# eanswer/TactileSimulation

Hardware: AMD Instinct MI355X
Metric: env-steps/sec (fwd+bwd) TactilePush batch=4096 (higher is better)
Workload: dtype f32

## Files before the change

include/tsim.h:

```cpp
#ifndef TSIM_H
#define TSIM_H
#include <stdint.h>
#ifdef __cplusplus
extern "C" {
#endif

typedef struct tsim_batch tsim_batch;
enum { TSIM_F32 = 0, TSIM_F64 = 1 };

int tsim_batch_create(const int32_t* I, const double* F, int B, int tape_capacity, int dtype, int device,
                      tsim_batch** out);
void tsim_batch_destroy(tsim_batch* b);

int tsim_ndof_r(const tsim_batch* b);
int tsim_ndof_u(const tsim_batch* b);
int tsim_ndof_var(const tsim_batch* b);
int tsim_ndof_tactile(const tsim_batch* b);
int tsim_batch_size(const tsim_batch* b);
int tsim_dtype(const tsim_batch* b);
double tsim_timestep(const tsim_batch* b);
int tsim_tape_len(const tsim_batch* b);

int tsim_update_model(tsim_batch* b, const int32_t* I, const double* F, void* stream);

// ... 53 lines not shown

int tsim_cache_save(tsim_batch* b, void* stream);
int tsim_cache_pop(tsim_batch* b, void* stream);
int tsim_cache_clear(tsim_batch* b);
int tsim_cache_reserve(tsim_batch* b, int depth);
int tsim_cache_depth(const tsim_batch* b);

int tsim_debug_eval(tsim_batch* b, const void* q1, const void* q0, const void* qd0, const void* u,
                    void* g_out, void* H_out, long long* cycles, void* stream);

int tsim_debug_signature(tsim_batch* b, int t_first, int n, uint32_t* out, void* stream);

int tsim_debug_stamps(tsim_batch* b, long long* cycles);

int tsim_launch_info(const tsim_batch* b, int32_t* out);
enum { TSIM_KT_FORWARD = 0, TSIM_KT_TAXELS = 1, TSIM_KT_BACKWARD = 2, TSIM_KT_COUNT = 3 };
int tsim_kernel_timing(tsim_batch* b, int enable);
int tsim_kernel_times(tsim_batch* b, double* ms_sum, int32_t* launches);
int tsim_set_lanes_per_env(tsim_batch* b, int lanes);
int tsim_static_model(const tsim_batch* b);
int tsim_set_static(tsim_batch* b, int allow);
const char* tsim_kernel_variant(const tsim_batch* b);
enum { TSIM_OPT_PAIR_CULL = 1, TSIM_OPT_VALUE_TRIALS = 2, TSIM_OPT_TRIAL_HELPERS = 3, TSIM_OPT_VALUE_FIRST = 4, TSIM_OPT_CROSS_KINKS = 5, TSIM_OPT_EVAL_BUDGET = 6,
       TSIM_OPT_ALL_DEFAULT = 7, TSIM_OPT_FRAME_RECORDS = 8, TSIM_OPT_FORWARD_SPLIT = 9, TSIM_OPT_PREDICTOR_HELPERS = 10 };
int tsim_set_option(tsim_batch* b, int option, int value);
int tsim_get_option(const tsim_batch* b, int option);

int tsim_last_evals(tsim_batch* b, int32_t* host_out);
int tsim_last_helper_trials(tsim_batch* b, int32_t* host_out);

#define TSIM_KINK_FACTOR 1000.0
#define TSIM_KINK_LS 4
#define TSIM_KINK_MAX 6
int tsim_set_solver_options(tsim_batch* b, int cross_kinks, int eval_budget);
int tsim_last_gnorm(tsim_batch* b, float* host_out);

const char* tsim_last_error(void);

#ifdef __cplusplus
}
#endif
#endif
```

tactilesimulation_amd/csrc/tsim_batch.h:

```cpp
#pragma once
#include <hip/hip_runtime.h>
#include <cstdint>
#include <string>
#include <vector>
#include "../../include/tsim.h"
#include "tsim_launch.h"

static thread_local std::string g_err;
static int fail(const std::string& m) { g_err = m; return 1; }
#define HIPCHK(x) do { hipError_t e_ = (x); if (e_ != hipSuccess) return fail(std::string(#x) + ": " + hipGetErrorString(e_)); } while (0)

struct DeviceGuard {
  int prev = -1; bool ok = true;
  explicit DeviceGuard(int dev) {
    if (hipGetDevice(&prev) != hipSuccess) prev = -1;
    if (prev != dev) ok = hipSetDevice(dev) == hipSuccess; else prev = -1;
  }
  ~DeviceGuard() { if (prev >= 0) (void)hipSetDevice(prev); }
};
#define TS_DEVICE(b) DeviceGuard guard_((b)->device); if (!guard_.ok) return fail("hipSetDevice(" + std::to_string((b)->device) + ") failed")

static bool capturing(hipStream_t st) {
  hipStreamCaptureStatus cs = hipStreamCaptureStatusNone;
  return hipStreamIsCapturing(st, &cs) != hipSuccess || cs != hipStreamCaptureStatusNone;
// ... 47 lines not shown
  int value_trials = 2;
  int pred_helpers = 1;
  int trial_helpers = 1;
  int value_first = 1;
  bool ab_no_episode_lpt = false, ab_inkernel_readout = false, ab_no_free_run = false, ab_lockstep = false, ab_taxels_per_record = false, ab_no_envtab_cpt = false, ab_no_default_opts = false, ab_inkernel_frame_out = false; int ab_bwd_lpe = 0, ab_lpt_deal = 2;
  int pair_cull = 1;
  int static_id = 0, static_exact = 0, env_struct_ok = 0, no_static = 0;
  DevBuf dKmask, dFlag;
  DevBuf fposeR, fposeD; int fpose_frames = 0;
  int pose_valid = 0;
  int pose_off = 0;
  int tt_off = 0;
  int tax_slots = 0;
  size_t esz;
  std::vector<CacheEntry> cache;
  std::vector<void*> pool;
  std::vector<void*> retired;
  long long* bwd_stamps = nullptr;
  void* dLdp = nullptr; DevBuf zbuf, pgpart; int pg_chunks = 0;
  int pg_groups = TS_PG_CONTACT; DevBuf pgbpart;
  DevBuf tan_src; size_t tan_src_reals = 0; int tan_src_captured = 0;
  DevBuf pg_slots;
  int adj_kernel = -1, adj_passes = 0;
  int kt_on = 0;
  std::vector<KtPair> kt;
  std::vector<hipEvent_t> kt_free;
};
template <class F> static auto by_real(const tsim_batch* b, F&& f) { return by_dtype(b->dtype, f); }
static void split_release(tsim_batch* b) {
  if (b->split_st) (void)hipStreamDestroy(b->split_st);
  if (b->split_fork) (void)hipEventDestroy(b->split_fork);
  if (b->split_join) (void)hipEventDestroy(b->split_join);
  b->split_st = nullptr; b->split_fork = b->split_join = nullptr;
}

struct KtScope {
  tsim_batch* b; hipStream_t st; KtPair p; bool on = false;
  KtScope(tsim_batch* b_, int kind, hipStream_t st_) : b(b_), st(st_) {
    if (!b->kt_on || b->kt.size() >= (size_t)1 << 16) return;
    if (capturing(st)) return;
    hipEvent_t e[2];
    for (int i = 0; i < 2; ++i) {
      if (!b->kt_free.empty()) { e[i] = b->kt_free.back(); b->kt_free.pop_back(); }
      else if (hipEventCreate(&e[i]) != hipSuccess) { (void)hipGetLastError(); if (i) b->kt_free.push_back(e[0]); return; }
    }
    p.a = e[0]; p.b = e[1]; p.kind = kind;
// ... 27 lines not shown
```

tactilesimulation_amd/csrc/tsim_env_push.h:

```cpp
#pragma once

template <class R>
__global__ void __launch_bounds__(256) k_push_action(int B, const R* __restrict__ u, const R* __restrict__ ext, R* __restrict__ a) {
  const int i = blockIdx.x * 256 + threadIdx.x;
  if (i >= B * 6) return;
  const int e = i / 6, c = i - e * 6;
  a[i] = c < 3 ? (R)tanh((double)u[e * 3 + c]) : (c < 5 ? ext[e * 2 + c - 3] : (R)0);
}

template <class R>
__global__ void __launch_bounds__(256) k_push_action_bwd(int B, const R* __restrict__ u, const R* __restrict__ da, R* __restrict__ du) {
  const int i = blockIdx.x * 256 + threadIdx.x;
  if (i >= B * 3) return;
  const int e = i / 3, c = i - e * 3;
  const double t = tanh((double)u[i]);
  du[i] = (R)((double)da[e * 6 + c] * (1.0 - t * t));
}

template <class R>
__global__ void __launch_bounds__(256) k_push_observe(int B, int ntac, const R* __restrict__ q, const R* __restrict__ var,
                                                      const R* __restrict__ tac, const R* __restrict__ goal, const R* __restrict__ u,
                                                      R* __restrict__ obs, R* __restrict__ rew) {
  const int W = 3 + ntac;
  const long long i = (long long)blockIdx.x * 256 + threadIdx.x;
// ... 145 lines not shown
  if (pol->obs_mode == TSIM_PUSH_OBS_TACTILE && (!tac0 || !tac_out)) return fail("push_closed_rollout: tac0 and tac_out are required with the tactile observation (they feed it)");
  if (b->record && b->t_cur + (long long)num_frames * num_steps > b->cap) return fail("push_closed_rollout: tape capacity exceeded (" + std::to_string(b->cap) + " sub-steps)");
  TS_DEVICE(b);
  if (int rc = by_real(b, [&](auto r) { return push_closed_rollout_t<decltype(r)>(b, pol, goal, dist, tac0, num_frames, num_steps, q_out, qd_out, var_out, tac_out, u_out, gl_out, h1_out, h2_out, status, (hipStream_t)stream); })) return rc;
  if (b->record) b->t_cur += num_frames * num_steps;
  b->has_prev = 1;
  return 0;
}

template <class R>
static int push_closed_backward_t(tsim_batch* b, const tsim_push_policy* pol, const void* goal, int nframes, int nsub, const void* df_dq, const void* df_dvar,
                                  const void* du_direct, const void* u_out, const void* h1_out, const void* h2_out, void* g1_out, void* g2_out, void* g3_out,
                                  void* dobs_tac, void* df_du, hipStream_t st) {
  BwdArgs<R> a = bwd_args<R>(b);
  a.n = nframes * nsub; a.seed_stride = nsub; a.frames = 1;
  a.df_dq = (const R*)df_dq; a.df_dvar = (const R*)df_dvar; a.df_du = (R*)df_du;
  a.pol = make_push_policy<R>(pol);
  a.pol.goal = (const R*)goal; a.pol.du_direct = (const R*)du_direct;
  a.pol.u_out = (R*)u_out; a.pol.h1_out = (R*)h1_out; a.pol.h2_out = (R*)h2_out;
  a.pol.g1_out = (R*)g1_out; a.pol.g2_out = (R*)g2_out; a.pol.g3_out = (R*)g3_out; a.pol.dobs_tac = (R*)dobs_tac;
  if (!ts_launch<true, R>(ts_plan(b, b->dLdp ? TS_K_CLOSED_BACKWARD_Z : TS_K_BACKWARD, true, 0), st, a, (R*)b->zbuf)) return fail("no closed-loop k_backward instantiation for the launch plan");
  HIPCHK(hipGetLastError());
  b->adj_kernel = b->dLdp ? TSIM_ADJ_CLOSED_BACKWARD_Z : TSIM_ADJ_BACKWARD;
  if (!b->dLdp) { b->adj_passes = 0; return 0; }
  const R* seeds = nullptr;
  if (a.pol.mode == TSIM_PUSH_OBS_TACTILE && (b->pg_groups & TS_PG_CONTACT)) {
    if (nframes > b->cap || !b->pg_slots) return fail("push_closed_backward: the seed table is missing or too small");
    ts_closed_slots_launch(b->pg_slots, nframes, st);
    HIPCHK(hipGetLastError());
    seeds = (const R*)dobs_tac + (size_t)b->B * PP_NTAC;
  }
  return launch_param_passes<R>(b, a.n, nsub, 1, seeds ? (const int32_t*)b->pg_slots : nullptr, seeds, st);
}

extern "C" int tsim_push_closed_backward(tsim_batch* b, const tsim_push_policy* pol, const void* goal, int num_frames, int num_steps,
                                         const void* df_dq, const void* df_dvar, const void* du_direct, const void* u_out, const void* h1_out, const void* h2_out,
                                         void* g1_out, void* g2_out, void* g3_out, void* dobs_tac, void* df_du, void* stream) {
  if (int rc = push_closed_check(b, pol, num_frames, num_steps, "push_closed_backward")) return rc;
  if (!pol->W1p || !pol->W2 || pol->w1_stride < push_obs_len(pol->obs_mode) || pol->w1_stride % 4 || pol->w1_stride > 64 * (int)PP_OCH) return fail("push_closed_backward: W1p [64][w1_stride >= observation length, multiple of 4] and W2 are required");
  if (!b->record) return fail("push_closed_backward: reset(backward_flag=True) was not called");
  long long n;
  if (int rc = taped_window(b, "push_closed_backward", num_frames, num_steps, &n)) return rc;
  if (!goal || !du_direct || !u_out || !h1_out || !h2_out || !g1_out || !g2_out || !g3_out) return fail("push_closed_backward: null pointer");
  if (pol->obs_mode == TSIM_PUSH_OBS_TACTILE && !dobs_tac) return fail("push_closed_backward: dobs_tac is required with the tactile observation");
  TS_DEVICE(b);
  if (int rc = by_real(b, [&](auto r) { return push_closed_backward_t<decltype(r)>(b, pol, goal, num_frames, num_steps, df_dq, df_dvar, du_direct, u_out, h1_out, h2_out, g1_out, g2_out, g3_out, dobs_tac, df_du, (hipStream_t)stream); })) return rc;
// ... 48 lines not shown
```

tactilesimulation_amd/csrc/tsim_hip.hip:

```cpp
#include <hip/hip_runtime.h>
#include <cstdio>
#include <cstdlib>
#include <cstring>
#include <cmath>
#include <algorithm>
#include <string>
#include <vector>
#include "../../include/tsim.h"
#include "tsim_eval.h"
#include "tsim_policy_push.h"
#include "tsim_static_pusher.h"


#include "tsim_kernels.h"
#include "tsim_param_grad.h"
#include "tsim_launch.h"
#include "tsim_batch.h"

__global__ void __launch_bounds__(1024) k_order_by_evals(const int* evals, int* order, int B, int ns, int lo, int span, int deal) {
  __shared__ int hist[64], base[64];
  const int t = threadIdx.x;
  if (t < 64) hist[t] = 0;
  __syncthreads();
  auto bin = [lo, span](int ev) { return min(max((ev - lo) * 64 / span, 0), 63); };
  for (int e = t; e < B; e += 1024) atomicAdd(&hist[bin(evals[e])], 1);
  __syncthreads();
  if (t == 0) { int acc = 0; for (int k = 63; k >= 0; --k) { base[k] = acc; acc += hist[k]; } }
  __syncthreads();
  const int nwaves = (B + ns - 1) / ns;
  for (int e = t; e < B; e += 1024) {
    const int r = atomicAdd(&base[bin(evals[e])], 1);
    int w = r % nwaves;
    const int sl = r / nwaves;
    if ((deal == 1 && (sl & 1)) || (deal == 2 && sl > 0)) w = nwaves - 1 - w;
    order[w * ns + sl] = e;
  }
}

template <class R> struct ReadArgs { const int* I; const R* F; const R* Fenv; int fstride; int B, t0; const R* tape; R* var_out; R* poseR; double* poseD; int nspt; int stage_cpt; int tk; };
// ... 748 lines not shown
template <class R>
static int launch_param_passes(tsim_batch* b, int n, int seed_stride, int frames, const int32_t* tac_slot, const void* df_dtac, hipStream_t st) {
  b->adj_passes = 0;
  if (!b->dLdp) return 0;
  if (b->pg_groups & TS_PG_CONTACT) {
    if (launch_param_grad<R>(b, n, seed_stride, frames, tac_slot, df_dtac, st)) return 1;
    b->adj_passes |= 1;
  }
  if (b->pg_groups & ~TS_PG_CONTACT) {
    if (launch_param_grad_body<R>(b, n, st)) return 1;
    b->adj_passes |= 2;
  }
  return 0;
}

template <class R>
static int launch_backward(tsim_batch* b, int n, int seed_stride, int frames, const int32_t* tac_slot, const void* df_dq, const void* df_dvar, const void* df_dtac, void* df_du, hipStream_t st) {
  BwdArgs<R> a = bwd_args<R>(b);
  a.n = n; a.seed_stride = seed_stride; a.frames = frames; a.tac_slot = tac_slot;
  a.df_dq = (const R*)df_dq; a.df_dvar = (const R*)df_dvar; a.df_dtac = (const R*)df_dtac; a.df_du = (R*)df_du; a.cyc = b->bwd_stamps;
  {
    KtScope kt_(b, TSIM_KT_BACKWARD, st);
    const TsPlan plan = ts_plan(b, b->dLdp ? TS_K_BACKWARD_Z : TS_K_BACKWARD, false, b->ab_bwd_lpe);
    if (!ts_launch<false, R>(plan, st, a, (R*)b->zbuf)) return fail("no k_backward instantiation for the launch plan");
  }
  HIPCHK(hipGetLastError());
  b->adj_kernel = b->dLdp ? TSIM_ADJ_BACKWARD_Z : TSIM_ADJ_BACKWARD;
  return launch_param_passes<R>(b, n, seed_stride, frames, tac_slot, df_dtac, st);
}

static SlotPlan tangent_plan(const tsim_batch* b, int ndir, bool with_dtab, int kernel = TS_K_TANGENT) {
  const int nhist = b->I[TSIM_IH_INTEGRATOR] == 2 ? 4 : 2, P = with_dtab ? ts_pg_count(b->I[TSIM_IH_NPAIR], b->I[TSIM_IH_NSENSOR], b->nr) : 0;
  return slot_block_plan(b, ts_plan(b, kernel, false, 0), 0, ts_tan_slot_reals(b->nr, b->nu, P, nhist, ndir));
}
template <class R>
static void tangent_args(const tsim_batch* b, TanArgs<R>& a, int T, int S, int ndir, const int32_t* tac_slot, const void* du, const void* dq0, const void* dqd0, const void* dtab,
                         void* dq_out, void* dqd_out, void* dvar_out, void* dtac_out) {
  a.I = b->dI; a.F = (const R*)b->dF; a.Fenv = (const R*)b->dFenv; a.fstride = b->nfrec;
  a.B = b->B; a.n = T * S; a.t_end = b->t_cur; a.nsub = S; a.nframes = T; a.ndir = ndir; a.tk = b->tape_k;
  a.stage_cpt = b->stage_cpt; a.cull = b->pair_cull; a.tac_slot = tac_slot; a.tape = (const R*)b->tape;
  a.du = (const R*)du; a.dq0 = (const R*)dq0; a.dqd0 = (const R*)dqd0; a.dtab = (const R*)dtab;
  a.dq_out = (R*)dq_out; a.dqd_out = (R*)dqd_out; a.dvar_out = (R*)dvar_out; a.dtac_out = (R*)dtac_out;
}
template <class R>
static int launch_tangent_body_src(tsim_batch* b, TanArgs<R>& a, hipStream_t st, const char* who) {
  if (!a.dtab || !(b->pg_groups & ~TS_PG_CONTACT)) return 0;
  const int ndir = a.ndir;
// ... 176 lines not shown
  {
    int cus = 0;
    if (hipDeviceGetAttribute(&cus, hipDeviceAttributeMultiprocessorCount, device) != hipSuccess || cus <= 0) cus = 256;
    b->n_simd = 4 * cus;
  }
  b->stage_cpt = 0;
  detect_static_model(b);
  b->tape_k = kernel_mode(b, b->lpe_forced) != TS_KM_GENERIC ? 1 : 0;
  b->rec = ts_rec(nr, nu, (int)b->esz, b->tape_k);
  if (lds_bytes_for(b, 1) > 64 * 1024) { delete b; return fail("model needs more than 64 KiB of LDS per environment"); }
  decide_stage_cpt(b);
  b->nspt = b->I[TSIM_IH_NSPRIM];
  size_t tape_bytes = (size_t)(tape_capacity + 1) * B * b->rec * b->esz;
  if (hipMalloc(&b->dI, (b->I.size() + b->nsched) * sizeof(int32_t)) != hipSuccess || hipMalloc(&b->dF, b->F.size() * b->esz) != hipSuccess ||
      hipMalloc(&b->tape, tape_bytes) != hipSuccess || hipMalloc(&b->lamq, (size_t)2 * B * nr * b->esz) != hipSuccess ||
      hipMalloc(&b->lamv, (size_t)2 * B * nr * b->esz) != hipSuccess || hipMalloc(&b->evals, (size_t)B * sizeof(int)) != hipSuccess || hipMalloc((void**)&b->helped, (size_t)B * sizeof(int)) != hipSuccess || hipMemset(b->helped, 0, (size_t)B * sizeof(int)) != hipSuccess || hipMalloc((void**)&b->gnorm, (size_t)B * sizeof(float)) != hipSuccess || hipMalloc(&b->order, (size_t)B * sizeof(int)) != hipSuccess || hipMalloc((void**)&b->order_ep, (size_t)B * sizeof(int)) != hipSuccess || hipMalloc(&b->prev, (size_t)B * 2 * nr * sizeof(double)) != hipSuccess ||
      (b->nspt > 0 && (hipMalloc(&b->poseR, (size_t)B * b->nspt * TP_R_SIZE * b->esz) != hipSuccess || hipMalloc((void**)&b->poseD, (size_t)B * b->nspt * TP_D_SIZE * sizeof(double)) != hipSuccess))) {
    tsim_batch_destroy(b);
    return fail("hipMalloc failed (tape bytes = " + std::to_string(tape_bytes) + ")");
  }
  if (hipMemset(b->tape, 0, tape_bytes) != hipSuccess || hipMemset(b->lamq, 0, (size_t)2 * B * nr * b->esz) != hipSuccess ||
      hipMemset(b->lamv, 0, (size_t)2 * B * nr * b->esz) != hipSuccess) { tsim_batch_destroy(b); return fail("hipMemset failed"); }
  if (upload_model(b, nullptr)) { tsim_batch_destroy(b); return 1; }
  if (B >= 64 && !getenv("TSIM_NO_FORWARD_SPLIT")) {
    if (hipStreamCreateWithFlags(&b->split_st, hipStreamNonBlocking) != hipSuccess || hipEventCreateWithFlags(&b->split_fork, hipEventDisableTiming) != hipSuccess ||
        hipEventCreateWithFlags(&b->split_join, hipEventDisableTiming) != hipSuccess) {
      (void)hipGetLastError();
      split_release(b);
    }
  }
  *out = b;
  return 0;
}

void tsim_batch_destroy(tsim_batch* b) {
  if (!b) return;
  DeviceGuard guard_(b->device);
  for (auto& e : b->cache) (void)hipFree(e.buf);
  for (void* p : b->pool) (void)hipFree(p);
  for (void* p : b->retired) (void)hipFree(p);
  for (auto& k : b->kt) { (void)hipEventDestroy(k.a); (void)hipEventDestroy(k.b); }
  for (hipEvent_t e : b->kt_free) (void)hipEventDestroy(e);
  split_release(b);
  (void)hipFree(b->tape);
  delete b;
}
// ... 47 lines not shown
  if (lanes != 0 && lanes != 16 && lanes != 32 && lanes != 64) return fail("set_lanes_per_env: 0 (automatic), 16, 32 or 64");
  b->lpe_forced = lanes;
  shape_changed(b);
  return 0;
}
int tsim_static_model(const tsim_batch* b) { return kernel_mode(b, b->lpe_forced) != TS_KM_GENERIC ? b->static_id : 0; }
const char* tsim_kernel_variant(const tsim_batch* b) {
  const int km = kernel_mode(b, b->lpe_forced);
  if (km == TS_KM_STATIC) return "static:pusher";
  if (km == TS_KM_PARAM) return "param:pusher";
  return "generic";
}
int tsim_set_static(tsim_batch* b, int allow) {
  b->no_static = allow ? 0 : 1;
  shape_changed(b);
  return 0;
}
int tsim_set_option(tsim_batch* b, int option, int value) {
  if (option == TSIM_OPT_PAIR_CULL) { b->pair_cull = value != 0; return 0; }
  if (option == TSIM_OPT_VALUE_TRIALS) { if (value < 0) return fail("set_option: TSIM_OPT_VALUE_TRIALS >= 0"); b->value_trials = value; return 0; }
  if (option == TSIM_OPT_TRIAL_HELPERS) { b->trial_helpers = value != 0; return 0; }
  if (option == TSIM_OPT_VALUE_FIRST) { b->value_first = value != 0; return 0; }
  if (option == TSIM_OPT_PREDICTOR_HELPERS) { b->pred_helpers = value != 0; return 0; }
  return fail("set_option: unknown option " + std::to_string(option));
}
int tsim_get_option(const tsim_batch* b, int option) {
  if (option == TSIM_OPT_PAIR_CULL) return b->pair_cull;
  if (option == TSIM_OPT_VALUE_TRIALS) return b->value_trials;
  if (option == TSIM_OPT_TRIAL_HELPERS) return b->trial_helpers;
  if (option == TSIM_OPT_VALUE_FIRST) return b->value_first;
  if (option == TSIM_OPT_CROSS_KINKS) return b->cross_kinks;
  if (option == TSIM_OPT_EVAL_BUDGET) return b->eval_budget;
  if (option == TSIM_OPT_ALL_DEFAULT) return default_options(b) ? 1 : 0;
  if (option == TSIM_OPT_FRAME_RECORDS) return b->last_frame_rec;
  if (option == TSIM_OPT_FORWARD_SPLIT) return b->last_fwd_split;
  if (option == TSIM_OPT_PREDICTOR_HELPERS) return b->pred_helpers;
  return -1;
}
int tsim_set_solver_options(tsim_batch* b, int cross_kinks, int eval_budget) {
  if (eval_budget < 0) return fail("set_solver_options: negative evaluation budget");
  b->cross_kinks = cross_kinks != 0;
  b->eval_budget = eval_budget;
  return 0;
}
int tsim_last_gnorm(tsim_batch* b, float* host_out) {
  TS_DEVICE(b);
  if (hipMemcpy(host_out, b->gnorm, (size_t)b->B * sizeof(float), hipMemcpyDeviceToHost) != hipSuccess) return fail("last_gnorm: copy failed");
  return 0;
}
int tsim_last_helper_trials(tsim_batch* b, int32_t* host_out) {
  TS_DEVICE(b);
  if (hipMemcpy(host_out, b->helped, (size_t)b->B * sizeof(int), hipMemcpyDeviceToHost) != hipSuccess) return fail("last_helper_trials: copy failed");
  return 0;
}
int tsim_last_evals(tsim_batch* b, int32_t* host_out) {
  TS_DEVICE(b);
  if (hipMemcpy(host_out, b->evals, (size_t)b->B * sizeof(int), hipMemcpyDeviceToHost) != hipSuccess) return fail("last_evals: copy failed");
  return 0;
}
// ... 369 lines not shown
```

tactilesimulation_amd/csrc/tsim_kernels.h:

```cpp
#pragma once
#include <hip/hip_runtime.h>
#include "../../include/tsim.h"
#include "tsim_eval.h"
#include "tsim_policy_push.h"

template <class MS, class C> __device__ __forceinline__ int ts_integrator(const C& c) {
  if constexpr (std::is_void<MS>::value) return ts_u(c.I[TSIM_IH_INTEGRATOR]); else return MS::Iv(TSIM_IH_INTEGRATOR);
}
template <class MS> constexpr int ts_static_nr() { if constexpr (std::is_void<MS>::value) return 0; else return MS::Iv(TSIM_IH_NR); }

__host__ __device__ inline int ts_qw(int esz) { return 8 / esz; }
__host__ __device__ inline int ts_rec(int nr, int nu, int esz, int tk) { return (ts_qw(esz) * nr + nr + nr * nr + nu + (tk ? nr * nr : 0) + 1) & ~1; }
template <class R> __device__ __forceinline__ double* rec_q(R* rec) { return reinterpret_cast<double*>(rec); }
template <class R> __device__ __forceinline__ const double* rec_q(const R* rec) { return reinterpret_cast<const double*>(rec); }
template <class R> __device__ __forceinline__ int rec_qd(int nr) { return ts_qw((int)sizeof(R)) * nr; }
template <class R> __device__ __forceinline__ int rec_H(int nr) { return ts_qw((int)sizeof(R)) * nr + nr; }
template <class R> __device__ __forceinline__ int rec_u(int nr) { return ts_qw((int)sizeof(R)) * nr + nr + nr * nr; }
template <class R> __device__ __forceinline__ int rec_K(int nr, int nu) { return ts_qw((int)sizeof(R)) * nr + nr + nr * nr + nu; }

template <int LPE, class R>
__device__ __forceinline__ void readout(const Ctx<R>& c, int lane, int env, bool wr_var, bool wr, bool has_var, bool has_tac, R* var_out, R* tac_out, int tb = 0, int te = 0x7fffffff) {
  if (has_var && wr_var) {
    for (int e = lane; e < c.nvar; e += LPE) {
      const int l = c.I[c.off_var + e * TSIM_VI_SIZE + TSIM_VI_LINK];
// ... 705 lines not shown
        for (int e = 0; e < 12; ++e) sq_ += g[e] * T[e];
        c.lamq[lane] += sq_;
      }
      pair_stage_tangent(c, pk, 0, lane, R(1), 1);
      if (lane < nr) {
        const R* T = c.PT + lane * PT_SIZE;
        R sv_ = R(0);
#pragma unroll
        for (int e = 6; e < 12; ++e) sv_ += g[e] * T[e];
        c.lamv[lane] += sv_;
      }
    }
  }
  TS_SYNC();
}

#ifdef TS_BWD_TWO_WAVES
#define TS_KLB_BWD __launch_bounds__(TS_WAVE)
#else
#define TS_KLB_BWD TS_KLB
#endif
template <class R, int NRM, bool EXPJ, int LPE, bool POLICY = false, class MS = void>
__global__ void TS_KLB_BWD k_backward(BwdArgs<R> a) {
  constexpr bool SAVEZ = false; R* const zsave = nullptr;
#include "tsim_kernels_backward.h"
}
template <class R, int NRM, bool EXPJ, int LPE, bool POLICY = false, class MS = void>
__global__ void TS_KLB_BWD k_backward_z(BwdArgs<R> a, R* zsave) {
  constexpr bool SAVEZ = true;
#include "tsim_kernels_backward.h"
}
template <class R, int NRM, bool EXPJ, int LPE, class MS = void>
__global__ void TS_KLB_BWD k_closed_backward_z(BwdArgs<R> a, R* zsave) {
  constexpr bool POLICY = true, SAVEZ = true;
#include "tsim_kernels_backward.h"
}


template <class R, int LPE, class MS, int SN, int J>
__device__ __forceinline__ void ts_vjp_sprim(const Ctx<R>& c, int lane, const TsLinkState<R>* st, const S6<R>& Wk, const R* wtac, R& dlq, R& dlv) {
  using T = TsTopo<MS>;
  constexpr int so = MS::Iv(TSIM_IH_OFF_SENSOR) + SN * TSIM_SI_SIZE, nsp = MS::Iv(so + TSIM_SI_NSPRIM);
  if constexpr (J < nsp) {
    constexpr int pk = MS::Iv(MS::Iv(TSIM_IH_OFF_SPRIM) + MS::Iv(so + TSIM_SI_SPRIM0) + J);
    constexpr int o = MS::Iv(TSIM_IH_OFF_PAIR) + pk * TSIM_PI_SIZE, prim = MS::Iv(o + TSIM_PI_PRIM), la = MS::Iv(o + TSIM_PI_LINKA), lb = MS::Iv(o + TSIM_PI_LINKB);
    const int t0 = ts_u(c.I[c.off_sensor + SN * TSIM_SI_SIZE + TSIM_SI_TAX0]), nt = ts_u(c.I[c.off_sensor + SN * TSIM_SI_SIZE + TSIM_SI_NTAX]);
    R pf[TSIM_PF_SIZE], sf[TSIM_SF_SIZE];
#pragma unroll
    for (int e = 0; e < TSIM_SF_SIZE; ++e) sf[e] = ts_F<R, MS>(c, MS::Iv(TSIM_IH_FOFF_SENSOR) + SN * TSIM_SF_SIZE + e);
    M3<R> RP; V3<R> pP; PairPose<R> P; S6<R> Vrel, dVA, dVB;
    ts_fused_pair_pose<R, MS, pk>(c, st, pf, RP, pP, P, Vrel, dVA, dVB);
    R g[12];
    const bool any_live = vjp_taxels<LPE, R, prim>(c, lane, t0, nt, prim, pf + TSIM_PF_SHAPE, sf, P, wtac, g);
    if (any_live) {
      seg_sum_many<LPE, 12>(g);
      const int k = lane;
      constexpr int ancA = la != 0 ? T::li(la == 0 ? 1 : la, TSIM_LI_ANCMASK) : 0, ancB = lb != 0 ? T::li(lb == 0 ? 1 : lb, TSIM_LI_ANCMASK) : 0;
// ... 88 lines not shown
```

tactilesimulation_amd/csrc/tsim_kernels_backward.h:

```cpp
  extern __shared__ __attribute__((aligned(16))) unsigned char smem_raw[];
  R* lds = reinterpret_cast<R*>(smem_raw);
  constexpr int NS = TS_WAVE / LPE;
  const int slot = threadIdx.x / LPE, lane = threadIdx.x % LPE;
  const bool valid = (int)blockIdx.x * NS + slot < a.B;
  const int env = min((int)blockIdx.x * NS + slot, a.B - 1);
  Ctx<R> c; ctx_init<R, MS>(c, a.I, a.F, lds, NS, slot, lane, LPE, a.stage_cpt != 0, a.Fenv ? a.Fenv + (size_t)env * a.fstride : nullptr);
  c.cull = a.cull;
  const int nr = c.nr, nu = c.nu, REC = ts_rec(nr, nu, (int)sizeof(R), a.tk);
  const int nvar3 = 3 * c.nvar, ntac3 = 3 * c.ntax;
  R* H2 = c.H2;
  init_world(c, lane, LPE);
  if (a.cyc && blockIdx.x == 0) c.stamps = a.cyc;
  if (lane < nr) { c.lamq[lane] = a.lamq[(size_t)env * nr + lane]; c.lamv[lane] = a.lamv[(size_t)env * nr + lane]; }
  const bool bdf2_model = ts_integrator<MS>(c) == 2;
  const size_t half = (size_t)a.B * nr;
  R lq1 = R(0), lv1 = R(0);
  if (bdf2_model && lane < nr) { lq1 = a.lamq[half + (size_t)env * nr + lane]; lv1 = a.lamv[half + (size_t)env * nr + lane]; }
  TS_SYNC();
  R du_frame = R(0);
  R pol_dq = R(0); bool pol_have = false;
  constexpr bool kFused = ts_static_fused<MS, R>();
  constexpr int NHL = (NRM * NRM + LPE - 1) / LPE;
  const int oqd = rec_qd<R>(nr), oH = rec_H<R>(nr), ou = rec_u<R>(nr), oK = rec_K<R>(nr, nu);
  double pq1 = 0.0, pq0 = 0.0; R pqd1 = R(0), pqd0 = R(0), pqdm = R(0), pu = R(0), pH[NHL];
  R pK[kFused ? NHL : 1];
  R* KT = c.H;
  {
    const R* r1 = a.tape + ((size_t)a.t_end * a.B + env) * REC;
    const R* r0 = a.tape + ((size_t)(a.t_end - 1) * a.B + env) * REC;
    if (lane < nr) { pq1 = rec_q(r1)[lane]; pqd1 = r1[oqd + lane]; pq0 = rec_q(r0)[lane]; pqd0 = r0[oqd + lane]; }
    if (bdf2_model && a.t_end >= 2 && lane < nr) pqdm = a.tape[((size_t)(a.t_end - 2) * a.B + env) * REC + oqd + lane];
    if (lane < nu) pu = r1[ou + lane];
#pragma unroll
    for (int i = 0; i < NHL; ++i) { const int e = lane + i * LPE; pH[i] = e < nr * nr ? r1[oH + e] : R(0); }
    if constexpr (kFused) {
#pragma unroll
      for (int i = 0; i < NHL; ++i) { const int e = lane + i * LPE; pK[i] = (a.tk && e < nr * nr) ? r1[oK + e] : R(0); }
    }
  }
  for (int j = a.n - 1; j >= 0; --j) {
    const int t = a.t_end - (a.n - 1 - j);
    const bool bdf2 = bdf2_model && t >= 2;
    c.cv = bdf2 ? R(1.5) / c.h : R(1) / c.h;
    c.ca = bdf2 ? R(2.25) / (c.h * c.h) : R(1) / (c.h * c.h);
    if (lane < nr) {
      c.qD[lane] = pq1; c.q[lane] = (R)pq1; c.q0[lane] = (R)pq0; c.qd0[lane] = pqd0;
      c.qd[lane] = pqd1;
      c.qa[lane] = bdf2 ? (R(3) * pqd1 - R(4) * pqd0 + pqdm) / (R(2) * c.h) : (pqd1 - pqd0) / c.h;
    }
    if (lane < nu) c.u[lane] = pu;
#pragma unroll
    for (int i = 0; i < NHL; ++i) { const int e = lane + i * LPE; if (e < nr * nr) H2[e] = pH[i]; }
    if constexpr (kFused) {
#pragma unroll
      for (int i = 0; i < NHL; ++i) { const int e = lane + i * LPE; if (e < nr * nr) KT[e] = pK[i]; }
    }
    TS_STAMP(c);
    if (j > 0) {
      const R* r1 = a.tape + ((size_t)(t - 1) * a.B + env) * REC;
      const R* r0 = a.tape + ((size_t)(t - 2) * a.B + env) * REC;
      pq1 = pq0; pqd1 = pqd0;
      if (lane < nr) { pq0 = rec_q(r0)[lane]; pqd0 = r0[oqd + lane]; }
      if (bdf2_model && t >= 3 && lane < nr) pqdm = a.tape[((size_t)(t - 3) * a.B + env) * REC + oqd + lane];
      if (lane < nu) pu = r1[ou + lane];
#pragma unroll
      for (int i = 0; i < NHL; ++i) { const int e = lane + i * LPE; pH[i] = e < nr * nr ? r1[oH + e] : R(0); }
      if constexpr (kFused) {
#pragma unroll
        for (int i = 0; i < NHL; ++i) { const int e = lane + i * LPE; pK[i] = (a.tk && e < nr * nr) ? r1[oK + e] : R(0); }
      }
    }
    __builtin_amdgcn_sched_barrier(0);
    TS_SYNC();
    TS_STAMP(c);
    const bool seeded = (j + 1) % a.seed_stride == 0;
    if constexpr (kFused) { }
    else if constexpr (std::is_void<MS>::value) phase1<R, true, EXPJ>(c, lane, R(1), R(0), R(0));
    else phase1_static_levels<R, MS, true>(c, lane, R(1), R(0), R(0));
    TS_STAMP(c);
    if (seeded) {
      const int fr = j / a.seed_stride;
      const size_t so = a.frames ? (size_t)fr * a.B + env : (size_t)env * (a.n / a.seed_stride) + fr;
      const int tslot = (a.frames && a.tac_slot) ? a.tac_slot[fr] : 0;
      const size_t sot = (a.frames && a.tac_slot) ? (size_t)max(tslot, 0) * a.B + env : so;
      if (a.df_dq && lane < nr) c.lamq[lane] += a.df_dq[so * nr + lane];
      if (POLICY && pol_have && lane < nr) c.lamq[lane] += pol_dq;
      TS_SYNC();
      const R* wtac_ = (a.df_dtac && ntac3 && tslot >= 0) ? a.df_dtac + sot * ntac3 : nullptr;
      if (POLICY) wtac_ = (pol_have && a.pol.mode == TSIM_PUSH_OBS_TACTILE) ? a.pol.dobs_tac + ((size_t)(fr + 1) * a.B + env) * PP_NTAC : nullptr;
      if constexpr (kFused) ts_static_output_vjp<R, LPE, MS>(c, lane, (a.df_dvar && nvar3) ? a.df_dvar + so * nvar3 : nullptr, wtac_);
      else output_vjp<LPE>(c, lane, (a.df_dvar && nvar3) ? a.df_dvar + so * nvar3 : nullptr, wtac_);
    }
    TS_STAMP(c);
#ifdef TS_BWD_REEVAL
    if (lane < nr) {
      c.qp[lane] = c.q0[lane] + c.h * c.qd0[lane]; c.qdp[lane] = c.qd0[lane];
      c.dl[lane] = (R)(c.qD[lane] - (double)c.qp[lane]); c.qpD[lane] = c.qD[lane] - (double)c.dl[lane];
    }
    TS_SYNC();
    evaluate<R, NRM, EXPJ, LPE, MS>(c, lane, R(1), c.cv, c.ca, true);
    for (int e = lane; e < nr * nr; e += LPE) {
      const R h_ = c.H[e];
      if constexpr (kFused) KT[e] = H2[e];
      H2[e] = h_;
    }
    TS_SYNC();
#endif
    if (lane < nr) c.rhs[lane] = c.lamq[lane] + c.cv * c.lamv[lane];
    TS_SYNC();
    solve_newton<R, NRM, LPE, double, ts_static_nr<MS>()>(H2, c.rhs, c.z, nr, true, lane);
    TS_STAMP(c);
    R ym, yq = R(0);
    if constexpr (!kFused) {
// ... 61 lines not shown
```

tactilesimulation_amd/host/batch.py:

```python
import ctypes as C

import numpy as np
import torch

from . import capi
from ..model import blob as _blob
from ..model.compiler import CompiledModel, load_model


def _ptr(t):
    return C.c_void_p(t.data_ptr()) if t is not None else None


class BatchSim:
    def __init__(self, model, batch_size, device="cuda:0", dtype=torch.float32, tape_capacity=512):
        if isinstance(model, str):
            model = load_model(model)
        assert isinstance(model, CompiledModel)
        self.model = model
        self.device = torch.device(device)
        if self.device.type != "cuda":
            raise RuntimeError("BatchSim needs a GPU device (got %s); the HIP path has no CPU fallback" % device)
        if dtype not in (torch.float32, torch.float64):
            raise ValueError("dtype must be float32 or float64")
# ... 338 lines not shown
        capi.check(capi.lib().tsim_last_gnorm(self._h, out.ctypes.data_as(C.POINTER(C.c_float))))
        return out

    def set_solver_options(self, cross_kinks=None, eval_budget=0):
        if cross_kinks is None:
            cross_kinks = self.dtype == torch.float32
        capi.check(capi.lib().tsim_set_solver_options(self._h, int(bool(cross_kinks)), int(eval_budget)))

    def set_lanes_per_env(self, lanes):
        capi.check(capi.lib().tsim_set_lanes_per_env(self._h, int(lanes)))

    def static_model(self):
        return capi.lib().tsim_static_model(self._h)

    def set_static(self, allow):
        capi.check(capi.lib().tsim_set_static(self._h, int(bool(allow))))

    def kernel_variant(self):
        return capi.lib().tsim_kernel_variant(self._h).decode()

    OPT_PAIR_CULL, OPT_VALUE_TRIALS, OPT_TRIAL_HELPERS, OPT_VALUE_FIRST, OPT_CROSS_KINKS, OPT_EVAL_BUDGET, OPT_ALL_DEFAULT, OPT_FRAME_RECORDS = 1, 2, 3, 4, 5, 6, 7, 8
    OPT_FORWARD_SPLIT = 9
    OPT_PREDICTOR_HELPERS = 10

    def set_option(self, option, value):
        capi.check(capi.lib().tsim_set_option(self._h, int(option), int(value)))

    def get_option(self, option):
        return capi.lib().tsim_get_option(self._h, int(option))

    KERNEL_KINDS = ("k_forward", "k_taxels", "k_backward")

    def kernel_timing(self, enable=True):
        capi.check(capi.lib().tsim_kernel_timing(self._h, int(bool(enable))))

    def kernel_times(self):
        ms, n = (C.c_double * 3)(), (C.c_int32 * 3)()
        capi.check(capi.lib().tsim_kernel_times(self._h, ms, n))
        return {k: (float(ms[i]), int(n[i])) for i, k in enumerate(self.KERNEL_KINDS)}

    def launch_info(self):
        out = (C.c_int32 * 4)()
        capi.lib().tsim_launch_info(self._h, out)
        return {"lds_bytes": out[0], "threads": out[1], "blocks": out[2], "lanes_per_env": out[3]}

    def tangent_launch_info(self, ndir=8, with_dtables=True):
# ... 24 lines not shown
```

tactilesimulation_amd/host/buildhash.py:

```python
import hashlib
import os


def digest(paths, flags=()):
    h = hashlib.sha256()
    for f in flags:
        h.update(f.encode() + b"\0")
    for p in paths:
        h.update(os.path.basename(p).encode() + b"\0")
        with open(p, "rb") as fh:
            h.update(fh.read())
    return h.hexdigest()


def sidecar(lib):
    return lib + ".buildhash"


def read(lib):
    try:
        return open(sidecar(lib)).read().strip()
    except OSError:
        return None

# ... 3 lines not shown
        fh.write(value + "\n")


_PKG = os.path.dirname(os.path.dirname(os.path.abspath(__file__)))
CSRC = os.path.join(_PKG, "csrc")
INCLUDE = os.path.join(os.path.dirname(_PKG), "include")
HIP_SO = os.path.join(CSRC, "libtsim_hip.so")
HIP_FLAGS = ["--offload-arch=gfx950", "-Os", "-std=c++17", "-fPIC", "-fno-slp-vectorize", "-mllvm", "-amdgpu-function-calls=false",
             "-mllvm", "-amdgpu-sched-strategy=iterative-ilp"]
HIP_UNITS = [("tsim_hip.hip", []), ("tsim_static_pusher.hip", ["-ffinite-math-only", "-fno-signed-zeros", "-O2"]),
             ("tsim_param_pusher.hip", ["-ffinite-math-only", "-fno-signed-zeros", "-O2"]),
             ("tsim_static_pusher_policy.hip", ["-ffinite-math-only", "-fno-signed-zeros"]),
             ("tsim_param_pusher_policy.hip", ["-ffinite-math-only", "-fno-signed-zeros"]),
             ("tsim_param_grad.hip", []),
             ("tsim_param_grad_body.hip", []),
             ("tsim_closed_backward_z.hip", []),
             ("tsim_tangent.hip", []),
             ("tsim_tangent_body.hip", []),
             ("tsim_tangent_closed.hip", []),
             ("tsim_frame_jacobian.hip", []),
             ("tsim_tactile_jacobian.hip", []),
             ("tsim_param_jacobian.hip", []),
             ("tsim_tactile_normal.hip", []),
             ("tsim_model.cpp", ["-ffp-contract=off"])]
HOST_FLAGS = ["-O2", "-std=c++17", "-fPIC"]


def hip_build_commands(hipcc, out_so=None):
    out_so = out_so or HIP_SO
    bdir = os.path.join(CSRC, "build")
    cmds, objs = [], []
    for src, extra in HIP_UNITS:
        obj = os.path.join(bdir, os.path.splitext(src)[0] + ".o")
        cmds.append(([hipcc] + (HIP_FLAGS if src.endswith(".hip") else HOST_FLAGS) + extra + ["-c", os.path.join(CSRC, src), "-o", obj], CSRC))
        objs.append(obj)
    cmds.append(([hipcc, "--offload-arch=gfx950", "-shared", "-fPIC", "-o", out_so] + objs, CSRC))
    return bdir, cmds


def hip_sources():
    srcs = sorted(f for f in os.listdir(CSRC) if f.endswith((".hip", ".h", ".cpp")))
    return [os.path.join(CSRC, f) for f in srcs] + [os.path.join(INCLUDE, f) for f in ("tsim.h", "tsim_blob.h", "tsim_env.h", "tsim_model.h")]


def hip_digest():
    return digest(hip_sources(), HIP_FLAGS + HOST_FLAGS + [u + ":" + " ".join(f) for u, f in HIP_UNITS])
# ... 31 lines not shown
                name = g("name")
                if not name:
                    continue
                name = name.group(1)
                rec = {k: int(g(k).group(1)) for k in ("agpr_count", "vgpr_count", "sgpr_count", "vgpr_spill_count", "sgpr_spill_count", "group_segment_fixed_size",
                                                        "private_segment_fixed_size", "max_flat_workgroup_size") if g(k)}
                rec["code_bytes"] = size.get(name)
                table[name] = rec
        with open(out, "w") as fh:
            json.dump(table, fh, indent=0, sort_keys=True)
        return table
    finally:
        shutil.rmtree(tmp, ignore_errors=True)


def kernel_name(kernel, dtype, nr, has_exp, lanes, variant, policy=False, default_opts=False):
    nrm, expj, lpe = (16, True, 64) if has_exp else ((8 if nr <= 8 else 16), False, lanes)
    if variant != "generic":
        nrm = 8
    ms = {"generic": ("v", "void"), "static:pusher": ("14TsStaticPusher", "TsStaticPusher"), "param:pusher": ("7TsParamI14TsStaticPusherE", "TsParam<TsStaticPusher>")}[variant]
    if default_opts and kernel == "k_forward" and variant != "generic" and dtype == "f32" and lpe == 16:
        ms = ("13TsDefaultOptsI%sE" % ms[0], "TsDefaultOpts<%s>" % ms[1])
    r = {"f32": ("f", "float"), "f64": ("d", "double")}[dtype]
    if kernel == "k_frame_records":
        return ("_Z15k_frame_recordsI%sLi%dE%sEv7FwdArgsIT_Ei10TsSubRange" % (r[0], lpe, ms[0]), "k_frame_records<%s, LPE=%d, %s>" % (r[1], lpe, ms[1]))
    if kernel == "k_forward_fr":
        return ("_Z12k_forward_frI%sLi%dELi%dE%sEv7FwdArgsIT_E" % (r[0], nrm, lpe, ms[0]), "k_forward_fr<%s, NRM=%d, LPE=%d, %s>" % (r[1], nrm, lpe, ms[1]))
    if kernel == "k_closed_backward_z":
        back = {"generic": 1, "static:pusher": 2, "param:pusher": 4}[variant]
        return ("_Z19k_closed_backward_zI%sLi%dELb%dELi%dE%sEv7BwdArgsIT_EPS%d_" % (r[0], nrm, int(expj), lpe, ms[0], back),
                "k_closed_backward_z<%s, NRM=%d, EXPJ=%s, LPE=%d, %s>" % (r[1], nrm, str(expj).lower(), lpe, ms[1]))
    args = {"k_forward": "7FwdArgs", "k_backward": "7BwdArgs"}[kernel]
    mangled = "_Z%d%sI%sLi%dELb%dELi%dELb%dE%sEv%sIT_E" % (len(kernel), kernel, r[0], nrm, int(expj), lpe, int(policy), ms[0], args)
    return mangled, "%s<%s, NRM=%d, EXPJ=%s, LPE=%d, POLICY=%s, %s>" % (kernel, r[1], nrm, str(expj).lower(), lpe, str(policy).lower(), ms[1])
```

Before: 35.65 million.

## Precompute per-frame output VJP seeds in a parallel prepass before backward sweep

Adds a k_adjoint_seeds kernel that computes the static output VJP (variable and tactile adjoint seeds) for every frame and env in parallel from the tape. A k_backward_pre variant of the backward kernel then adds those precomputed seeds instead of evaluating ts_static_output_vjp inside the serial reverse time loop. It is enabled by default for f32 fused static/param pusher plans with frames==1 and no param grads. The cost is an extra kernel launch, a seed buffer sized tape_capacity*B*2*nr, and extra global traffic to write and read the seeds.

```diff
diff --git a/include/tsim.h b/include/tsim.h
--- a/include/tsim.h
+++ b/include/tsim.h
@@ -99,7 +99,7 @@
 int tsim_set_static(tsim_batch* b, int allow);
 const char* tsim_kernel_variant(const tsim_batch* b);
 enum { TSIM_OPT_PAIR_CULL = 1, TSIM_OPT_VALUE_TRIALS = 2, TSIM_OPT_TRIAL_HELPERS = 3, TSIM_OPT_VALUE_FIRST = 4, TSIM_OPT_CROSS_KINKS = 5, TSIM_OPT_EVAL_BUDGET = 6,
-       TSIM_OPT_ALL_DEFAULT = 7, TSIM_OPT_FRAME_RECORDS = 8, TSIM_OPT_FORWARD_SPLIT = 9, TSIM_OPT_PREDICTOR_HELPERS = 10 };
+       TSIM_OPT_ALL_DEFAULT = 7, TSIM_OPT_FRAME_RECORDS = 8, TSIM_OPT_FORWARD_SPLIT = 9, TSIM_OPT_PREDICTOR_HELPERS = 10, TSIM_OPT_ADJOINT_PREPASS = 11 };
 int tsim_set_option(tsim_batch* b, int option, int value);
 int tsim_get_option(const tsim_batch* b, int option);
 
diff --git a/tactilesimulation_amd/csrc/tsim_adjoint_pre.h b/tactilesimulation_amd/csrc/tsim_adjoint_pre.h
--- /dev/null
+++ b/tactilesimulation_amd/csrc/tsim_adjoint_pre.h
@@ -0,0 +1,76 @@
+#pragma once
+#include "tsim_launch.h"
+
+__host__ __device__ inline int ts_ap_tab_reals(int nfrec, int nslot, bool env_tables) { return ((env_tables ? nslot : 1) * (nfrec + 2) + 3) & ~3; }
+__host__ __device__ inline int ts_ap_slot_reals(int esz) { return 8 * (8 / esz) + 5 * 8; }
+__host__ __device__ inline size_t ts_ap_lds_bytes(int nfrec, int nslot, bool env_tables, int esz) {
+  return (size_t)(ts_ap_tab_reals(nfrec, nslot, env_tables) + nslot * ts_ap_slot_reals(esz)) * esz;
+}
+
+template <class R, int LPE, class MS>
+__global__ void __launch_bounds__(TS_WAVE) __attribute__((amdgpu_waves_per_eu(MS::PARAM ? 3 : 4))) k_adjoint_seeds(BwdArgs<R> a, R* sseed) {
+  using T = TsTopo<MS>;
+  static_assert(T::NR <= 8 && T::NR <= LPE, "k_adjoint_seeds: eight reals per slot array");
+  extern __shared__ __attribute__((aligned(16))) unsigned char smem_raw[];
+  R* lds = reinterpret_cast<R*>(smem_raw);
+  constexpr int NS = TS_WAVE / LPE, nr = T::NR, nu = MS::Iv(TSIM_IH_NU), nfrec = MS::Iv(TSIM_IH_FOFF_CPT);
+  const int slot = threadIdx.x / LPE, lane = threadIdx.x % LPE;
+  const long long total = (long long)(a.n / a.seed_stride) * a.B, item0 = (long long)blockIdx.x * NS + slot;
+  const bool valid = item0 < total;
+  const long long item = valid ? item0 : total - 1;
+  const int fr = (int)(item / a.B), env = (int)(item % a.B);
+  Ctx<R> c{};
+  R* mf = lds;
+  if (a.Fenv) {
+    mf += slot * (nfrec + 2);
+    const R* Fe = a.Fenv + (size_t)env * a.fstride;
+    for (int i = lane; i < nfrec; i += LPE) mf[i] = Fe[i];
+  } else {
+    for (int i = threadIdx.x; i < nfrec; i += TS_WAVE) mf[i] = a.F[i];
+  }
+  TS_SYNC();
+  c.I = a.I; c.LI = a.I; c.F = mf; c.Fg = a.F; c.cull = a.cull;
+  c.nl = MS::Iv(TSIM_IH_NL); c.nr = nr; c.nu = nu; c.nvar = MS::Iv(TSIM_IH_NVAR); c.npair = MS::Iv(TSIM_IH_NPAIR); c.ncpt = MS::Iv(TSIM_IH_NCPT);
+  c.nsensor = MS::Iv(TSIM_IH_NSENSOR); c.ntax = a.I[TSIM_IH_NTAXEL]; c.nd = nr;
+  c.off_link = MS::Iv(TSIM_IH_OFF_LINK); c.off_dof = MS::Iv(TSIM_IH_OFF_DOF); c.off_motor = MS::Iv(TSIM_IH_OFF_MOTOR); c.off_var = MS::Iv(TSIM_IH_OFF_VAR);
+  c.off_pair = MS::Iv(TSIM_IH_OFF_PAIR); c.off_sensor = MS::Iv(TSIM_IH_OFF_SENSOR); c.off_sprim = MS::Iv(TSIM_IH_OFF_SPRIM);
+  c.foff_link = MS::Iv(TSIM_IH_FOFF_LINK); c.foff_dof = MS::Iv(TSIM_IH_FOFF_DOF); c.foff_motor = MS::Iv(TSIM_IH_FOFF_MOTOR); c.foff_var = MS::Iv(TSIM_IH_FOFF_VAR);
+  c.foff_pair = MS::Iv(TSIM_IH_FOFF_PAIR); c.foff_sensor = MS::Iv(TSIM_IH_FOFF_SENSOR); c.foff_cpt = nfrec; c.foff_tax = MS::Iv(TSIM_IH_FOFF_TAXEL);
+  c.h = mf[TSIM_FH_H]; c.gx = mf[TSIM_FH_GX]; c.gy = mf[TSIM_FH_GY]; c.gz = mf[TSIM_FH_GZ]; c.tol = mf[TSIM_FH_TOL];
+  c.cv = R(1) / c.h; c.ca = R(1) / (c.h * c.h);
+  {
+    R* p = lds + ts_ap_tab_reals(nfrec, NS, a.Fenv != nullptr) + slot * ts_ap_slot_reals((int)sizeof(R));
+    c.qD = reinterpret_cast<double*>(p); p += 8 * (8 / (int)sizeof(R));
+    c.q = p; p += 8; c.qd = p; p += 8; c.qa = p; p += 8; c.lamq = p; p += 8; c.lamv = p;
+  }
+  const int j = (fr + 1) * a.seed_stride - 1, t = a.t_end - (a.n - 1 - j);
+  const int REC = ts_rec(nr, nu, (int)sizeof(R), a.tk), oqd = rec_qd<R>(nr);
+  const R* r1 = a.tape + ((size_t)t * a.B + env) * REC;
+  const R* r0 = a.tape + ((size_t)(t - 1) * a.B + env) * REC;
+  if (lane < nr) {
+    const double q1 = rec_q(r1)[lane];
+    const R qd1 = r1[oqd + lane], qd0 = r0[oqd + lane];
+    c.qD[lane] = q1; c.q[lane] = (R)q1; c.qd[lane] = qd1; c.qa[lane] = (qd1 - qd0) / c.h;
+    c.lamq[lane] = R(0); c.lamv[lane] = R(0);
+  }
+  TS_SYNC();
+  const int nvar3 = 3 * c.nvar, ntac3 = 3 * c.ntax;
+  const size_t so = (size_t)fr * a.B + env;
+  const int tslot = a.tac_slot ? a.tac_slot[fr] : 0;
+  const size_t sot = a.tac_slot ? (size_t)max(tslot, 0) * a.B + env : so;
+  const R* wtac = (a.df_dtac && ntac3 && tslot >= 0) ? a.df_dtac + sot * ntac3 : nullptr;
+  ts_static_output_vjp<R, LPE, MS>(c, lane, (a.df_dvar && nvar3) ? a.df_dvar + so * nvar3 : nullptr, wtac);
+  if (valid && lane < nr) {
+    R* o = sseed + (size_t)item * (2 * nr);
+    o[lane] = c.lamq[lane]; o[nr + lane] = c.lamv[lane];
+  }
+}
+
+template <class R, int NRM, bool EXPJ, int LPE, class MS>
+__global__ void TS_KLB_BWD k_backward_pre(BwdArgs<R> a, const R* sseed) {
+  constexpr bool POLICY = false, SAVEZ = false, PRE = true; R* const zsave = nullptr;
+  static_assert(ts_static_fused<MS, R>(), "k_backward_pre: a fused compiled-in model");
+#include "tsim_kernels_backward.h"
+}
+
+bool ts_adjoint_pre_launch(const TsPlan& plan, hipStream_t st, const BwdArgs<float>& a, float* sseed, int nfrec);
diff --git a/tactilesimulation_amd/csrc/tsim_adjoint_pre.hip b/tactilesimulation_amd/csrc/tsim_adjoint_pre.hip
--- /dev/null
+++ b/tactilesimulation_amd/csrc/tsim_adjoint_pre.hip
@@ -0,0 +1,20 @@
+#include <hip/hip_runtime.h>
+#include "tsim_adjoint_pre.h"
+
+template <class MS>
+static void adjoint_pre_launch(const TsPlan& plan, hipStream_t st, const BwdArgs<float>& a, float* sseed, int nfrec) {
+  constexpr int LPE = 16, NS = TS_WAVE / LPE;
+  const long long items = (long long)(a.n / a.seed_stride) * a.B;
+  if (items > 0) {
+    const size_t lds = ts_ap_lds_bytes(nfrec, NS, a.Fenv != nullptr, (int)sizeof(float));
+    hipLaunchKernelGGL((k_adjoint_seeds<float, LPE, MS>), dim3((unsigned)((items + NS - 1) / NS)), dim3(TS_WAVE), lds, st, a, sseed);
+  }
+  hipLaunchKernelGGL((k_backward_pre<float, 8, false, LPE, MS>), dim3(plan.grid), dim3(TS_WAVE), plan.lds, st, a, (const float*)sseed);
+}
+
+bool ts_adjoint_pre_launch(const TsPlan& plan, hipStream_t st, const BwdArgs<float>& a, float* sseed, int nfrec) {
+  if (plan.kernel != TS_K_BACKWARD || plan.policy || plan.lpe != 16 || plan.nrm != 8 || plan.expj || !plan.fused) return false;
+  if (plan.variant == TS_KM_STATIC) { adjoint_pre_launch<TsStaticPusher>(plan, st, a, sseed, nfrec); return true; }
+  if (plan.variant == TS_KM_PARAM) { adjoint_pre_launch<TsParamPusher>(plan, st, a, sseed, nfrec); return true; }
+  return false;
+}
diff --git a/tactilesimulation_amd/csrc/tsim_batch.h b/tactilesimulation_amd/csrc/tsim_batch.h
--- a/tactilesimulation_amd/csrc/tsim_batch.h
+++ b/tactilesimulation_amd/csrc/tsim_batch.h
@@ -93,6 +93,7 @@
   DevBuf tan_src; size_t tan_src_reals = 0; int tan_src_captured = 0;
   DevBuf pg_slots;
   int adj_kernel = -1, adj_passes = 0;
+  int adj_pre = 1, adj_pre_ran = 0; DevBuf sseed;
   int kt_on = 0;
   std::vector<KtPair> kt;
   std::vector<hipEvent_t> kt_free;
diff --git a/tactilesimulation_amd/csrc/tsim_env_push.h b/tactilesimulation_amd/csrc/tsim_env_push.h
--- a/tactilesimulation_amd/csrc/tsim_env_push.h
+++ b/tactilesimulation_amd/csrc/tsim_env_push.h
@@ -191,6 +191,7 @@
   if (!ts_launch<true, R>(ts_plan(b, b->dLdp ? TS_K_CLOSED_BACKWARD_Z : TS_K_BACKWARD, true, 0), st, a, (R*)b->zbuf)) return fail("no closed-loop k_backward instantiation for the launch plan");
   HIPCHK(hipGetLastError());
   b->adj_kernel = b->dLdp ? TSIM_ADJ_CLOSED_BACKWARD_Z : TSIM_ADJ_BACKWARD;
+  b->adj_pre_ran = 0;
   if (!b->dLdp) { b->adj_passes = 0; return 0; }
   const R* seeds = nullptr;
   if (a.pol.mode == TSIM_PUSH_OBS_TACTILE && (b->pg_groups & TS_PG_CONTACT)) {
diff --git a/tactilesimulation_amd/csrc/tsim_hip.hip b/tactilesimulation_amd/csrc/tsim_hip.hip
--- a/tactilesimulation_amd/csrc/tsim_hip.hip
+++ b/tactilesimulation_amd/csrc/tsim_hip.hip
@@ -15,6 +15,7 @@
 #include "tsim_kernels.h"
 #include "tsim_param_grad.h"
 #include "tsim_launch.h"
+#include "tsim_adjoint_pre.h"
 #include "tsim_batch.h"
 
 __global__ void __launch_bounds__(1024) k_order_by_evals(const int* evals, int* order, int B, int ns, int lo, int span, int deal) {
@@ -809,7 +810,12 @@
   {
     KtScope kt_(b, TSIM_KT_BACKWARD, st);
     const TsPlan plan = ts_plan(b, b->dLdp ? TS_K_BACKWARD_Z : TS_K_BACKWARD, false, b->ab_bwd_lpe);
-    if (!ts_launch<false, R>(plan, st, a, (R*)b->zbuf)) return fail("no k_backward instantiation for the launch plan");
+    b->adj_pre_ran = 0;
+    if constexpr (std::is_same<R, float>::value) {
+      if (b->adj_pre && b->sseed && frames == 1 && !b->dLdp && plan.fused && plan.lpe == 16 && b->I[TSIM_IH_INTEGRATOR] != 2 &&
+          ts_adjoint_pre_launch(plan, st, a, (float*)b->sseed, b->nfrec)) b->adj_pre_ran = 1;
+    }
+    if (!b->adj_pre_ran && !ts_launch<false, R>(plan, st, a, (R*)b->zbuf)) return fail("no k_backward instantiation for the launch plan");
   }
   HIPCHK(hipGetLastError());
   b->adj_kernel = b->dLdp ? TSIM_ADJ_BACKWARD_Z : TSIM_ADJ_BACKWARD;
@@ -1032,6 +1038,11 @@
   if (hipMemset(b->tape, 0, tape_bytes) != hipSuccess || hipMemset(b->lamq, 0, (size_t)2 * B * nr * b->esz) != hipSuccess ||
       hipMemset(b->lamv, 0, (size_t)2 * B * nr * b->esz) != hipSuccess) { tsim_batch_destroy(b); return fail("hipMemset failed"); }
   if (upload_model(b, nullptr)) { tsim_batch_destroy(b); return 1; }
+  b->adj_pre = getenv("TSIM_NO_ADJOINT_PREPASS") ? 0 : 1;
+  if (b->adj_pre && b->tape_k && dtype == TSIM_F32 && tape_capacity > 0 && hipMalloc(&b->sseed, (size_t)tape_capacity * B * 2 * nr * b->esz) != hipSuccess) {
+    (void)hipGetLastError();
+    b->adj_pre = 0;
+  }
   if (B >= 64 && !getenv("TSIM_NO_FORWARD_SPLIT")) {
     if (hipStreamCreateWithFlags(&b->split_st, hipStreamNonBlocking) != hipSuccess || hipEventCreateWithFlags(&b->split_fork, hipEventDisableTiming) != hipSuccess ||
         hipEventCreateWithFlags(&b->split_join, hipEventDisableTiming) != hipSuccess) {
@@ -1125,6 +1136,7 @@
   if (option == TSIM_OPT_TRIAL_HELPERS) { b->trial_helpers = value != 0; return 0; }
   if (option == TSIM_OPT_VALUE_FIRST) { b->value_first = value != 0; return 0; }
   if (option == TSIM_OPT_PREDICTOR_HELPERS) { b->pred_helpers = value != 0; return 0; }
+  if (option == TSIM_OPT_ADJOINT_PREPASS) { b->adj_pre = value != 0; return 0; }
   return fail("set_option: unknown option " + std::to_string(option));
 }
 int tsim_get_option(const tsim_batch* b, int option) {
@@ -1138,6 +1150,7 @@
   if (option == TSIM_OPT_FRAME_RECORDS) return b->last_frame_rec;
   if (option == TSIM_OPT_FORWARD_SPLIT) return b->last_fwd_split;
   if (option == TSIM_OPT_PREDICTOR_HELPERS) return b->pred_helpers;
+  if (option == TSIM_OPT_ADJOINT_PREPASS) return b->adj_pre_ran;
   return -1;
 }
 int tsim_set_solver_options(tsim_batch* b, int cross_kinks, int eval_budget) {
diff --git a/tactilesimulation_amd/csrc/tsim_kernels.h b/tactilesimulation_amd/csrc/tsim_kernels.h
--- a/tactilesimulation_amd/csrc/tsim_kernels.h
+++ b/tactilesimulation_amd/csrc/tsim_kernels.h
@@ -751,17 +751,17 @@
 #endif
 template <class R, int NRM, bool EXPJ, int LPE, bool POLICY = false, class MS = void>
 __global__ void TS_KLB_BWD k_backward(BwdArgs<R> a) {
-  constexpr bool SAVEZ = false; R* const zsave = nullptr;
+  constexpr bool SAVEZ = false, PRE = false; R* const zsave = nullptr; const R* const sseed = nullptr;
 #include "tsim_kernels_backward.h"
 }
 template <class R, int NRM, bool EXPJ, int LPE, bool POLICY = false, class MS = void>
 __global__ void TS_KLB_BWD k_backward_z(BwdArgs<R> a, R* zsave) {
-  constexpr bool SAVEZ = true;
+  constexpr bool SAVEZ = true, PRE = false; const R* const sseed = nullptr;
 #include "tsim_kernels_backward.h"
 }
 template <class R, int NRM, bool EXPJ, int LPE, class MS = void>
 __global__ void TS_KLB_BWD k_closed_backward_z(BwdArgs<R> a, R* zsave) {
-  constexpr bool POLICY = true, SAVEZ = true;
+  constexpr bool POLICY = true, SAVEZ = true, PRE = false; const R* const sseed = nullptr;
 #include "tsim_kernels_backward.h"
 }
 
diff --git a/tactilesimulation_amd/csrc/tsim_kernels_backward.h b/tactilesimulation_amd/csrc/tsim_kernels_backward.h
--- a/tactilesimulation_amd/csrc/tsim_kernels_backward.h
+++ b/tactilesimulation_amd/csrc/tsim_kernels_backward.h
@@ -38,6 +38,13 @@
       for (int i = 0; i < NHL; ++i) { const int e = lane + i * LPE; pK[i] = (a.tk && e < nr * nr) ? r1[oK + e] : R(0); }
     }
   }
+  [[maybe_unused]] R psq = R(0), psv = R(0);
+  if constexpr (PRE) {
+    if (a.n % a.seed_stride == 0 && lane < nr) {
+      const R* sp = sseed + ((size_t)((a.n - 1) / a.seed_stride) * a.B + env) * (2 * nr);
+      psq = sp[lane]; psv = sp[nr + lane];
+    }
+  }
   for (int j = a.n - 1; j >= 0; --j) {
     const int t = a.t_end - (a.n - 1 - j);
     const bool bdf2 = bdf2_model && t >= 2;
@@ -56,6 +63,13 @@
       for (int i = 0; i < NHL; ++i) { const int e = lane + i * LPE; if (e < nr * nr) KT[e] = pK[i]; }
     }
     TS_STAMP(c);
+    [[maybe_unused]] const R sq_now = psq, sv_now = psv;
+    if constexpr (PRE) {
+      if (j > 0 && j % a.seed_stride == 0 && lane < nr) {
+        const R* sp = sseed + ((size_t)((j - 1) / a.seed_stride) * a.B + env) * (2 * nr);
+        psq = sp[lane]; psv = sp[nr + lane];
+      }
+    }
     if (j > 0) {
       const R* r1 = a.tape + ((size_t)(t - 1) * a.B + env) * REC;
       const R* r0 = a.tape + ((size_t)(t - 2) * a.B + env) * REC;
@@ -88,7 +102,8 @@
       TS_SYNC();
       const R* wtac_ = (a.df_dtac && ntac3 && tslot >= 0) ? a.df_dtac + sot * ntac3 : nullptr;
       if (POLICY) wtac_ = (pol_have && a.pol.mode == TSIM_PUSH_OBS_TACTILE) ? a.pol.dobs_tac + ((size_t)(fr + 1) * a.B + env) * PP_NTAC : nullptr;
-      if constexpr (kFused) ts_static_output_vjp<R, LPE, MS>(c, lane, (a.df_dvar && nvar3) ? a.df_dvar + so * nvar3 : nullptr, wtac_);
+      if constexpr (PRE) { if (lane < nr) { c.lamq[lane] += sq_now; c.lamv[lane] += sv_now; } TS_SYNC(); }
+      else if constexpr (kFused) ts_static_output_vjp<R, LPE, MS>(c, lane, (a.df_dvar && nvar3) ? a.df_dvar + so * nvar3 : nullptr, wtac_);
       else output_vjp<LPE>(c, lane, (a.df_dvar && nvar3) ? a.df_dvar + so * nvar3 : nullptr, wtac_);
     }
     TS_STAMP(c);
diff --git a/tactilesimulation_amd/host/batch.py b/tactilesimulation_amd/host/batch.py
--- a/tactilesimulation_amd/host/batch.py
+++ b/tactilesimulation_amd/host/batch.py
@@ -384,6 +384,7 @@
     OPT_PAIR_CULL, OPT_VALUE_TRIALS, OPT_TRIAL_HELPERS, OPT_VALUE_FIRST, OPT_CROSS_KINKS, OPT_EVAL_BUDGET, OPT_ALL_DEFAULT, OPT_FRAME_RECORDS = 1, 2, 3, 4, 5, 6, 7, 8
     OPT_FORWARD_SPLIT = 9
     OPT_PREDICTOR_HELPERS = 10
+    OPT_ADJOINT_PREPASS = 11
 
     def set_option(self, option, value):
         capi.check(capi.lib().tsim_set_option(self._h, int(option), int(value)))
diff --git a/tactilesimulation_amd/host/buildhash.py b/tactilesimulation_amd/host/buildhash.py
--- a/tactilesimulation_amd/host/buildhash.py
+++ b/tactilesimulation_amd/host/buildhash.py
@@ -49,6 +49,7 @@
              ("tsim_tactile_jacobian.hip", []),
              ("tsim_param_jacobian.hip", []),
              ("tsim_tactile_normal.hip", []),
+             ("tsim_adjoint_pre.hip", ["-ffinite-math-only", "-fno-signed-zeros", "-O2"]),
              ("tsim_model.cpp", ["-ffp-contract=off"])]
 HOST_FLAGS = ["-O2", "-std=c++17", "-fPIC"]
 
@@ -126,6 +127,13 @@
     if default_opts and kernel == "k_forward" and variant != "generic" and dtype == "f32" and lpe == 16:
         ms = ("13TsDefaultOptsI%sE" % ms[0], "TsDefaultOpts<%s>" % ms[1])
     r = {"f32": ("f", "float"), "f64": ("d", "double")}[dtype]
+    if kernel == "k_adjoint_seeds":
+        back = {"static:pusher": 2, "param:pusher": 4}[variant]
+        return ("_Z15k_adjoint_seedsI%sLi%dE%sEv7BwdArgsIT_EPS%d_" % (r[0], lpe, ms[0], back), "k_adjoint_seeds<%s, LPE=%d, %s>" % (r[1], lpe, ms[1]))
+    if kernel == "k_backward_pre":
+        back = {"static:pusher": 2, "param:pusher": 4}[variant]
+        return ("_Z14k_backward_preI%sLi%dELb%dELi%dE%sEv7BwdArgsIT_EPKS%d_" % (r[0], nrm, int(expj), lpe, ms[0], back),
+                "k_backward_pre<%s, NRM=%d, EXPJ=%s, LPE=%d, %s>" % (r[1], nrm, str(expj).lower(), lpe, ms[1]))
     if kernel == "k_frame_records":
         return ("_Z15k_frame_recordsI%sLi%dE%sEv7FwdArgsIT_Ei10TsSubRange" % (r[0], lpe, ms[0]), "k_frame_records<%s, LPE=%d, %s>" % (r[1], lpe, ms[1]))
     if kernel == "k_forward_fr":
```

After: 37.00 million, median of 6. 3.8% higher.
